# SpectacularAI/HybVIO

Hardware: AMD Instinct MI355X
Metric: VIO frames/sec at 752x480 stereo, 200 KLT features; pyramid+KLT HBM GB/s (higher is better)
Workload: dtype u8/int16 pixels, int32/int64 sums, f32 solve (tracker); f64 (EKF); 1 GPU; C3: 752x480 stereo, 200 pts -- the whole frame chained on one stream per sequence: 2 pyramid builds, temporal LK from predicted positions, 2-point rotation RANSAC on its output, stereo LK, GFTT key points every 2nd frame (HIP tracker), then the HIP EKF from the device mean: 20 track visits (triangulation + prepareVisualUpdate + chi2 gate; track lengths 5 + Geometric(0.2) <= 21 stereo poses = 20 .~; sequences_per_gpu=4096, engines_per_gpu=4, parallelism=replicas x1 (no collective)

## Files before the change

hybvio_amd/csrc/vu_prepare.hip:

```cpp
#include <stdlib.h>

#include "ekf_device.hpp"

#pragma clang fp contract(fast)

namespace hv {
__device__ long long g_vu_stamp[40];
__device__ long long g_tri_stamp[64];
#ifdef HV_EKF_PHASE_STAMPS
#define VU_STAMP(i) do { if (blockIdx.x == 0 && threadIdx.x == 0) g_vu_stamp[i] = (long long)__builtin_readcyclecounter(); } while (0)
#define TRI_STAMP(i) do { if (blockIdx.x == 0 && threadIdx.x == 0) g_tri_stamp[i] = (long long)__builtin_readcyclecounter(); } while (0)
#else
#define VU_STAMP(i) do { } while (0)
#define TRI_STAMP(i) do { } while (0)
#endif
namespace {

constexpr int VT_LATENCY = 768, VT_THROUGHPUT = 384;
constexpr int MAXP_ALL = 42;
constexpr int MAXP_SMALL = 22;
constexpr int MAXP_REC = 24;
constexpr int MAXNP = 21;
constexpr int POSE_WORDS = 51;
constexpr int ITER_WORDS = 26;
// ... 246 lines not shown
    mv3(dd, col, mapped);
    const int dst = j < 7 ? j : j < 14 ? 7 * ind1 + (j - 7) : dDim;
    if (!(j < 7 && ind1 == 0)) {
#pragma unroll
        for (int r = 0; r < 3; ++r) s_dpfi[r * ncol + dst] = mapped[r];
    }
    if (tid == 0) {
#pragma unroll
        for (int k = 0; k < 3; ++k) { pfi[k] = ip3[k]; pfw[k] = pf[k]; }
#pragma unroll
        for (int r = 0; r < 3; ++r)
#pragma unroll
            for (int c = 0; c < 3; ++c) R0T[3 * r + c] = R0[3 * c + r];
        scal[1] = 0.0; scal[2] = 1e10;
        s_flag[0] = 0;
    }
}

template <int MAXP, bool LONG = false>
struct VuLds {
    static constexpr int MAXC = MAXP * 7 + 1, MOT_STRIDE = 13;
    static constexpr int MAXPAIRS = 14 * MAXP - 7;
    static constexpr int LONG_T = (HV_GATE_TIGHT_ROWS + 2) * HV_GATE_TIGHT_ROWS, LONG_HS = (7 * MAXNP + 1) * HV_GATE_TIGHT_ROWS;
    static_assert(LONG_T == 7224 && LONG_HS == 12432, "the long gate's areas as the kernels were measured with");
    static constexpr int TRAIL = 0, IT = TRAIL + MAXP * POSE_WORDS, DPFI = IT + MAXP * ITER_WORDS, FEAT = DPFI + 3 * MAXC,
                         SMALL = FEAT + MAXP * 4, DPF = SMALL + 64, P0 = DPF + MAXNP * 21, MOT = P0 + 7 * MAXP * 9 + 7 * 9,
                         OWN = MOT + MAXPAIRS * MOT_STRIDE, LIN = OWN + MAXC * 9, LIN_END = LIN + 3 * MAXP * 9 + 32,
                         INTS = (LONG && LONG_T + LONG_HS > LIN_END) ? LONG_T + LONG_HS : LIN_END,
                         TOTAL = INTS + (MAXNP + 3 + 4 + MAXC + 1) / 2 + 1;
    static_assert(!LONG || P0 <= LONG_T, "the sources of the Jacobian's factors must lie below the region they are copied to");
    static constexpr int HS_DOUBLES = INTS - P0, T_DOUBLES = P0;
    static constexpr size_t BYTES = sizeof(double) * TOTAL;
};
static_assert(VuLds<42, true>::BYTES <= LDS_CU_BYTES, "the long build must fit one CU's LDS");

template <int MAXP, bool LONG = false>
struct VuRecLds {
    static constexpr int MAXC = MAXP * 7 + 1, MOT_STRIDE = 13;
    static constexpr int LONG_T = VuLds<MAXP, LONG>::LONG_T, LONG_HS = VuLds<MAXP, LONG>::LONG_HS;
    static constexpr int TRAIL = 0, IT = 0, FEAT = IT + MAXP * ITER_WORDS, DPF = FEAT + MAXP * 4, DPFI = DPF + MAXP * 21, SMALL = DPFI + 4,
                         SMALL_END = SMALL + 64;
    static constexpr int SHORT_T = lds_stride(48 + 1) * 48, SHORT_HS = ((7 * (MAXP_REC / 2) + 1 + 3) & ~3) * 48;
    static_assert(SHORT_T == 2352 && SHORT_HS == 4224, "the short gate's areas as the kernels were measured with");
    static constexpr int P0 = LONG ? LONG_T : SHORT_T;
    static constexpr int MOT = P0, OWN = P0, LIN = P0;
    static constexpr int INTS = LONG ? LONG_T + LONG_HS : P0 + SHORT_HS;
    static constexpr int TOTAL = INTS + (MAXNP + 3 + 4 + MAXC + 1) / 2 + 1;
    static constexpr int HS_DOUBLES = INTS - P0, T_DOUBLES = P0;
    static_assert(SMALL_END <= P0, "the record's copies must fit in front of the staged Jacobian");
    static constexpr size_t BYTES = sizeof(double) * TOTAL;
};
static_assert(VuRecLds<MAXP_REC>::BYTES + 32 <= 42 * 1280, "three record-fed short-class gates per CU");

__device__ __forceinline__ void prepare_pose_part(const double *pose, const double *pfw, double *o)
{
    const double pt[3] = {pfw[0] - pose[0], pfw[1] - pose[1], pfw[2] - pose[2]};
    double pfc[3], ipH[3], dip[9];
    mv3(pose + 3, pt, pfc);
    inverse_depth(pfc, ipH, dip);
    o[16] = pfc[2] == 0 ? 1.0 : pfc[2] < 0 ? 2.0 : 0.0;
    o[14] = ipH[0]; o[15] = ipH[1];
#pragma unroll
    for (int r = 0; r < 2; ++r)
#pragma unroll
        for (int c = 0; c < 3; ++c) o[3 * r + c] = dip[3 * r] * pose[3 + c] + dip[3 * r + 1] * pose[6 + c] + dip[3 * r + 2] * pose[9 + c];
#pragma unroll
    for (int jq = 0; jq < 4; ++jq) {
        const double *dR = pose + 12 + 9 * jq;
        double a1[3], b1[3], b2[3];
        mv3(dR, pt, a1);
        mTv3(dR, pose + 48, b1);
        mv3(pose + 3, b1, b2);
#pragma unroll
        for (int r = 0; r < 2; ++r) o[6 + 4 * r + jq] = dip[3 * r] * (a1[0] + b2[0]) + dip[3 * r + 1] * (a1[1] + b2[1]) + dip[3 * r + 2] * (a1[2] + b2[2]);
    }
}

__device__ __forceinline__ bool vu_admission(const VuPrepareArgs &a, const int b, const size_t rec, const int np_rec, const bool no_track)
{
    const int tid = threadIdx.x;
    const bool quota_used = a.success_counter && a.success_counter[b] >= a.max_successful;
    if (a.spec_tracks > 0) {
        if ((int)blockIdx.y < a.cursor[b]) return true;
        if (!quota_used && a.epoch[rec] == a.success_counter[b]) return true;
    }
    if (a.np_hi > 0 && np_rec >= 2 && np_rec <= a.np && (np_rec < a.np_lo || np_rec > a.np_hi)) {
        if (tid == 0) {
            if (a.class_inactive && a.active) a.active[rec] = 0;
            if (a.long_list && np_rec > a.np_hi) a.long_list[atomicAdd(a.long_count, 1)] = (int)rec;
        }
        return true;
    }
    if (a.np_hi > 0 && a.np_lo > 2 && no_track) {
        if (a.class_inactive && a.active && tid == 0) a.active[rec] = 0;
        return true;
    }
    if (quota_used) {
        if (tid == 0) {
            a.status[2 * rec] = HV_TRI_NOT_VISITED; a.status[2 * rec + 1] = HV_TRI_NOT_VISITED;
            if (a.active) a.active[rec] = 0;
            if (a.gate_status) a.gate_status[rec] = 1;
            if (a.spec_tracks > 0) {
                if (a.chi2) a.chi2[rec] = 0.0;
                a.pf[3 * rec] = 0.0; a.pf[3 * rec + 1] = 0.0; a.pf[3 * rec + 2] = 0.0;
            }
        }
        return true;
    }
    if (no_track) {
        if (tid == 0) {
            a.status[2 * rec] = HV_TRI_NOT_VISITED; a.status[2 * rec + 1] = HV_TRI_NOT_VISITED;
            if (a.active) a.active[rec] = 0;
            if (a.gate_status) a.gate_status[rec] = 1;
            if (a.rows_out) a.rows_out[rec] = 0;
            if (a.spec_tracks > 0) a.epoch[rec] = a.success_counter[b];
        }
        return true;
    }
    return false;
}

template <int VT, int MAXP, int FUSED, bool MAP = false, bool REC = false>
__device__ __forceinline__ void vu_prepare_body(const VuPrepareArgs &a, const int bx )
{
    static_assert(!REC || (FUSED == 1 || FUSED == 3), "record-fed builds are gate builds");
    using Lay = std::conditional_t<REC, VuRecLds<MAXP, FUSED == 3>, VuLds<MAXP, FUSED == 3>>;
    constexpr int MOT_STRIDE = Lay::MOT_STRIDE;
    extern __shared__ __attribute__((aligned(16))) double vu_lds[];
// ... 310 lines not shown
        double *M = s_small + 40, *pf0 = s_small + 49;
        if (tid == 0 && !(MAP && map_track)) {
            int status = HV_TRI_OK;
            if (a.linear) {  }
            else if (!s_flag[0]) status = HV_TRI_NO_CONVERGENCE;
            else if (scal[1] < a.rcond_threshold) status = HV_TRI_BAD_COND;
            if (status == HV_TRI_OK && !a.linear) {
                double d[9], q[3], w[3], Ml[9];
                inverse_depth(pfi, q, d);
                mv3(R0T, q, w);
#pragma unroll
                for (int k = 0; k < 3; ++k) { pfw[k] = w[k] + p0[k]; pf0[k] = q[k]; }
                if (pfw[0] == p0[0] && pfw[1] == p0[1] && pfw[2] == p0[2]) status = HV_TRI_UNKNOWN_PROBLEM;
                mm3(R0T, d, Ml);
#pragma unroll
                for (int k = 0; k < 9; ++k) M[k] = Ml[k];
            }
            s_flag[1] = status;
            s_flag[2] = 0;
        }
        __syncthreads();
        status = s_flag[1];
        if (status == HV_TRI_OK) {
            if (tid < ncol && !a.linear) {
                const int j = tid;
                double u[3] = {0, 0, 0}, v[3];
                if (j >= 3 && j < 7) mTv3(s_trail + 12 + 9 * (j - 3), pf0, u);
                const double cur[3] = {s_dpfi[j], s_dpfi[ncol + j], s_dpfi[2 * ncol + j]};
                mv3(M, cur, v);
#pragma unroll
                for (int r = 0; r < 3; ++r) s_dpfi[r * ncol + j] = u[r] + v[r] + (j == r ? 1.0 : 0.0);
            }
            if (tid < nt) {
                const double *cur = s_trail + tid * POSE_WORDS;
                const double d[3] = {pfw[0] - cur[0], pfw[1] - cur[1], pfw[2] - cur[2]};
                if (cur[9] * d[0] + cur[10] * d[1] + cur[11] * d[2] < 0) atomicOr(&s_flag[2], 1);
            }
            __syncthreads();
            if (s_flag[2]) status = HV_TRI_BEHIND;
        }
        if (!(MAP && map_track)) {
            const double dx = pfw[0] - p0[0], dy = pfw[1] - p0[1], dz = pfw[2] - p0[2], depth = sqrt(dx * dx + dy * dy + dz * dz);
            if (depth < a.min_dist || depth > a.max_dist) status = HV_TRI_BAD_DEPTH;
        }
        with_derivatives = status == HV_TRI_OK;
        if (with_derivatives)
            for (int i = tid; i < n * 21; i += VT) {
                const int k = i / 21, e = i - 21 * k, r = e / 7, c = e - 7 * r;
                double v = s_dpfi[r * ncol + 7 * k + c];
                if (a.stereo) v += s_dpfi[r * ncol + 7 * (k + n) + c];
                s_dpf[i] = v;
            }
        VU_STAMP(28);
        if (tid < nt) prepare_pose_part(s_trail + tid * POSE_WORDS, pfw, s_it + tid * ITER_WORDS);
        __syncthreads();
        VU_STAMP(29);
    }
    auto sft_col = [&](int c) -> double { return REC ? s_dpfi[c] : s_dpfi[c * ncol + dDim]; };
    const int rows = 2 * nt;
    if constexpr (FUSED != 0) {
        int prep = 0;
        for (int i = 0; i < nt && prep == 0; ++i) prep = (int)s_it[i * ITER_WORDS + 16];
        const double pf_out[3] = {pfw[0], pfw[1], pfw[2]};
        if (!(status == HV_TRI_OK && prep == 0)) {
            if (tid == 0) {
                st_out[0] = status; st_out[1] = prep;
                if (a.active) a.active[rec] = 0;
                if (a.gate_status) a.gate_status[rec] = 1;
                if (a.chi2) a.chi2[rec] = 0.0;
                if (a.spec_tracks > 0) a.epoch[rec] = a.success_counter[b];
#pragma unroll
                for (int k = 0; k < 3; ++k) a.pf[3 * rec + k] = pf_out[k];
            }
            return;
        }
        if (tid == 0) {
            st_out[0] = HV_TRI_OK; st_out[1] = 0;
            if (a.active) a.active[rec] = 1;
#pragma unroll
            for (int k = 0; k < 3; ++k) a.pf[3 * rec + k] = pf_out[k];
        }
        constexpr bool STRUCT = FUSED == 3;
        constexpr bool STAGED = FUSED == 1;
        const int na = 7 * n + 1, na4 = (na + 3) & ~3, ti = (rows + 15) >> 4;
        int Rs = lds_stride(rows + 1);
        constexpr int T_CAP = FUSED == 3 ? Lay::LONG_T : Lay::T_DOUBLES, REGION = FUSED == 3 ? Lay::LONG_HS : Lay::HS_DOUBLES;
        if (STRUCT && Rs * rows > T_CAP) Rs = lds_stride_tight(rows + 1);
        const int nrp = 16 * ti;
        double *Hs = vu_lds + (FUSED == 3 ? Lay::LONG_T : Lay::P0);
        const int f4s = na, nslots_g = VT / ((na + 63) & ~63);
        double *f_O4 = Hs, *f_DV = f_O4 + 4 * rows, *f_F4 = f_DV + 7 * rows, *f_WF = f_F4 + 4 * f4s, *f_FA = f_WF + 4 * na,
               *f_DWF = f_FA + 4 * rows, *f_FWF = f_DWF + 4 * rows, *f_WFp = f_FWF + 16, *f_G = f_WFp + 3 * na * nslots_g;
        const int g_cap = REGION - (int)(f_G - Hs);
        int *s_acol = s_flag + 4;
        if (tid < na) {
            int col = SFT;
            if (tid < 7 * n) {
                const int q = tid / 7, comp = tid - 7 * q;
                int ip, io;
                pos_ori(s_idx[q], ip, io);
                col = comp < 3 ? ip + comp : io + comp - 3;
            }
            s_acol[tid] = col;
            a.acol[rec * a.na_max + tid] = col;
        }
        if constexpr (STRUCT) {
            if (tid < nt) {
                const double *o = s_it + tid * ITER_WORDS;
                double *o4 = f_O4 + 8 * tid, *dv = f_DV + 14 * tid;
#pragma unroll
                for (int c = 0; c < 3; ++c) { o4[c] = o[c]; o4[4 + c] = o[3 + c]; }
                o4[3] = a.est_shift ? -s_feat[4 * tid + 2] : 0.0; o4[7] = a.est_shift ? -s_feat[4 * tid + 3] : 0.0;
#pragma unroll
                for (int comp = 0; comp < 7; ++comp) {
                    dv[comp] = comp < 3 ? -o[comp] : o[6 + comp - 3];
// ... 121 lines not shown
            if (a.spec_tracks > 0) a.epoch[rec] = a.success_counter[b];
        }
        return;
    }
    double *H = a.H + rec * rows_max * N;
    int *s_colmap = reinterpret_cast<int *>(s_p0);
    for (int c = tid; c < N; c += VT) {
        int code = -1;
        for (int q = 0; q < n; ++q) {
            int ip, io;
            pos_ori(s_idx[q], ip, io);
            if (c >= ip && c < ip + 3) code = 8 * q + (c - ip);
            else if (c >= io && c < io + 4) code = 8 * q + 3 + (c - io);
        }
        s_colmap[c] = code;
    }
    __syncthreads();
    const unsigned inv_nt = (unsigned)((0x100000000ull + (unsigned)nt - 1) / (unsigned)nt);
    for (int w = tid; w < N * nt; w += VT) {
        const int c = (int)__umulhi((unsigned)w, inv_nt), i = w - c * nt;
        const int code = s_colmap[c], k = code >> 3, comp = code & 7;
        const bool sft = c == 19 && with_derivatives && a.est_shift;
        const double *o = s_it + i * ITER_WORDS;
        double h0 = 0.0, h1 = 0.0;
        if (code >= 0) {
            if (k == i % n) {
                if (comp < 3) { h0 = -o[comp]; h1 = -o[3 + comp]; }
                else { h0 = o[6 + comp - 3]; h1 = o[10 + comp - 3]; }
            }
            if (with_derivatives) {
                const double *dp = s_dpf + 21 * k + comp;
                h0 += o[0] * dp[0] + o[1] * dp[7] + o[2] * dp[14];
                h1 += o[3] * dp[0] + o[4] * dp[7] + o[5] * dp[14];
            }
        } else if (sft) {
            const double t0 = s_dpfi[dDim], t1 = s_dpfi[ncol + dDim], t2 = s_dpfi[2 * ncol + dDim];
            h0 = o[0] * t0 + o[1] * t1 + o[2] * t2 - s_feat[4 * i + 2];
            h1 = o[3] * t0 + o[4] * t1 + o[5] * t2 - s_feat[4 * i + 3];
        }
        if (MAP && map_track && c >= map_off && c < map_off + 3) { h0 += o[c - map_off]; h1 += o[3 + c - map_off]; }
        *reinterpret_cast<double2 *>(H + (size_t)c * rows + 2 * i) = double2{h0, h1};
    }
    if (tid < nt) {
        const double *o = s_it + tid * ITER_WORDS;
#pragma unroll
        for (int r = 0; r < 2; ++r) {
            const size_t e = rec * rows_max + 2 * tid + r;
            if (a.f) a.f[e] = o[14 + r];
            a.v[e] = (a.y ? a.y[e] : 0.0) - o[14 + r];
        }
    }
    VU_STAMP(30);
    if (tid == 0) {
        int prep = 0;
        for (int i = 0; i < nt && prep == 0; ++i) prep = (int)s_it[i * ITER_WORDS + 16];
        st_out[0] = status; st_out[1] = prep;
        if (a.active) a.active[rec] = ((status == HV_TRI_OK || (MAP && map_track)) && prep == 0) ? 1 : 0;
        if (a.gate_status) a.gate_status[rec] = 1;
        if (a.spec_tracks > 0) a.epoch[rec] = a.success_counter[b];
#pragma unroll
        for (int k = 0; k < 3; ++k) a.pf[3 * rec + k] = pfw[k];
    }
}

constexpr int TRI_ITW = 28;
struct TriLds {
    int trail, it, dpfi, feat, small, scr, lsum, tot, ints, total;
    __host__ __device__ TriLds(int ntm)
    {
        trail = 0; it = trail + ntm * POSE_WORDS; dpfi = it + ntm * TRI_ITW; feat = dpfi + 3 * (7 * ntm + 1);
        small = feat + 4 * ntm; scr = small + 72; lsum = scr + 7 * ntm * 9; tot = lsum + 32; ints = tot + 64;
        total = ints + (MAXNP + 3 + 4 + 1) / 2 + 1;
    }
};

__device__ __forceinline__ double strided_sum(const double *base, int stride, int n, int part, int parts)
{
    double a0 = 0.0, a1 = 0.0, a2 = 0.0, a3 = 0.0;
    int k = part;
    for (; k + 3 * parts < n; k += 4 * parts) {
        a0 += base[(size_t)k * stride]; a1 += base[(size_t)(k + parts) * stride];
        a2 += base[(size_t)(k + 2 * parts) * stride]; a3 += base[(size_t)(k + 3 * parts) * stride];
    }
    for (; k < n; k += parts) a0 += base[(size_t)k * stride];
    return (a0 + a1) + (a2 + a3);
}

template <int NT>
__device__ __forceinline__ void vu_tri_body(const VuPrepareArgs &a, const int b)
{
    extern __shared__ __attribute__((aligned(16))) double vu_lds[];
    const int tid = threadIdx.x;
    const size_t rec = (size_t)b;
    const int np_rec = __builtin_amdgcn_readfirstlane(a.np_rec ? a.np_rec[rec] : a.np);
    if (np_rec < 2 || np_rec > a.np) return;
    if (a.np_hi > 0 && (np_rec < a.np_lo || np_rec > a.np_hi)) return;
    if (a.success_counter && a.success_counter[b] >= a.max_successful) return;
    const int n = np_rec, ncam = a.stereo ? 2 : 1, nt = n * ncam, N = a.n;
    const int nt_max = a.np * ncam;
    const int dDim = nt * 7, ncol = dDim + 1;
    const int np_carve = a.np_hi > 0 && a.np_hi < a.np ? a.np_hi : a.np;
    const TriLds L(np_carve * ncam);
    double *s_trail = vu_lds + L.trail, *s_it = vu_lds + L.it, *s_dpfi = vu_lds + L.dpfi, *s_feat = vu_lds + L.feat;
    double *s_small = vu_lds + L.small, *s_scr = vu_lds + L.scr, *s_L = vu_lds + L.lsum, *s_tot = vu_lds + L.tot;
    int *s_idx = reinterpret_cast<int *>(vu_lds + L.ints), *s_flag = s_idx + MAXNP + 3;
    const double *m = a.m + (size_t)b * N;
    double *pfi = s_small, *pfw = s_small + 3, *R0T = s_small + 18, *scal = s_small + 36, *sums13 = s_small + 52;
    auto sync = [] { lds_barrier(); };
    TRI_STAMP(0);
    if (tid < n) s_idx[tid] = a.pose_index[rec * a.np + tid];
    if (tid < nt) {
#pragma unroll
        for (int k = 0; k < 2; ++k) {
            s_feat[4 * tid + k] = a.features[(rec * nt_max + tid) * 2 + k];
            s_feat[4 * tid + 2 + k] = a.velocities[(rec * nt_max + tid) * 2 + k];
        }
    }
    sync();
    TRI_STAMP(1);
    if (tid < nt) trail_pose_record(a, m, s_idx, tid, n, s_trail + tid * POSE_WORDS);
    for (int i = tid; i < 3 * ncol; i += NT) s_dpfi[i] = 0.0;
    sync();
    TRI_STAMP(2);
    const double *p0 = s_trail;
    const int ind1 = a.stereo ? nt / 2 - 1 : nt - 1;
    if (tid < 15) two_camera_start(a, tid, ind1, ncol, dDim, s_trail, s_feat, s_dpfi, pfi, pfw, R0T, scal, s_flag);
    sync();
    TRI_STAMP(3);
    const double *Lm = s_L;
    auto update_col = [&](int j, const double *own, bool is_sft, const double (&X)[9], const double (&step)[3]) {
        const double d0 = s_dpfi[j], d1 = s_dpfi[ncol + j], d2 = s_dpfi[2 * ncol + j];
        double v[9];
#pragma unroll
        for (int e = 0; e < 9; ++e) v[e] = (Lm[e] * d0 + Lm[9 + e] * d1) + Lm[18 + e] * d2;
        double dEe[3] = {v[0], v[1], v[2]}, dM[9] = {v[3], v[4], v[5], v[4], v[6], v[7], v[5], v[7], v[8]};
        if (!is_sft) {
#pragma unroll
            for (int k = 0; k < 3; ++k) dEe[k] += own[k];
            dM[0] += own[3]; dM[1] += own[4]; dM[2] += own[5]; dM[4] += own[6]; dM[5] += own[7]; dM[8] += own[8];
            dM[3] = dM[1]; dM[6] = dM[2]; dM[7] = dM[5];
        } else {
#pragma unroll
            for (int k = 0; k < 3; ++k) dEe[k] += Lm[27 + k];
        }
        double t1[3], t2[3], t3[3];
        mv3(dM, step, t1);
        mv3(X, t1, t2);
        mv3(X, dEe, t3);
#pragma unroll
        for (int r = 0; r < 3; ++r) s_dpfi[r * ncol + j] += t2[r] - t3[r];
    };
    constexpr int PARTS_L = NT >= 240 ? 8 : NT >= 120 ? 4 : 2;
    constexpr int PARTS_T = NT >= 252 ? 4 : NT >= 126 ? 2 : 1;
    const int NC = 4 * nt, NPp = 3 * (nt - 1), NQ = 4 * (nt - 1);
    for (int it = 0; it < a.gn_iters; ++it) {
#define TRI_IT_STAMP(k) do { if (it < 5) TRI_STAMP(4 + 10 * it + (k)); } while (0)
        TRI_IT_STAMP(0);
        if (tid < nt) {
            const double *cur = s_trail + tid * POSE_WORDS;
            double *o = s_it + tid * TRI_ITW;
            double C[9], t[3], d[3], h[3];
            mm3(cur + 3, R0T, C);
#pragma unroll
            for (int k = 0; k < 3; ++k) d[k] = p0[k] - cur[k];
            mv3(cur + 3, d, t);
            const double pfiab[3] = {pfi[0], pfi[1], 1.0};
            mv3(C, pfiab, h);
#pragma unroll
            for (int k = 0; k < 3; ++k) h[k] += pfi[2] * t[k];
            const double ih2 = 1.0 / h[2], ih2sq = ih2 * ih2;
#pragma unroll
            for (int k = 0; k < 9; ++k) o[k] = C[k];
#pragma unroll
            for (int k = 0; k < 3; ++k) { o[9 + k] = t[k]; o[12 + k] = h[k]; o[23 + k] = d[k]; }
            o[26] = ih2;
#pragma unroll
            for (int r = 0; r < 2; ++r) {
#pragma unroll
                for (int c = 0; c < 2; ++c) o[15 + 3 * r + c] = -ih2 * C[3 * r + c] + h[r] * ih2sq * C[6 + c];
                o[15 + 3 * r + 2] = -t[r] * ih2 + h[r] * ih2sq * t[2];
                o[21 + r] = s_feat[4 * tid + r] - h[r] * ih2;
            }
        }
        sync();
        TRI_IT_STAMP(1);
        if (tid < 52) {
            const int k = tid >> 2, part = tid & 3;
            const int r = k / 3, c = k - 3 * r;
            const int x0 = k < 9 ? 15 + r : k < 12 ? 15 + (k - 9) : 21, y0 = k < 9 ? 15 + c : 21;
            const int dx = k < 12 ? 3 : 1, dy = k < 9 ? 3 : 1;
            double acc = 0.0, acc2 = 0.0;
            int i = part;
            for (; i + 4 < nt; i += 8) {
                const double *o = s_it + i * TRI_ITW, *o2 = o + 4 * TRI_ITW;
                acc += o[x0] * o[y0] + o[x0 + dx] * o[y0 + dy];
                acc2 += o2[x0] * o2[y0] + o2[x0 + dx] * o2[y0 + dy];
            }
            if (i < nt) { const double *o = s_it + i * TRI_ITW; acc += o[x0] * o[y0] + o[x0 + dx] * o[y0 + dy]; }
            acc += acc2;
            acc += __shfl_xor(acc, 1);
            acc += __shfl_xor(acc, 2);
            if (part == 0) sums13[k] = acc;
        }
        {
            const int t0 = NT > 64 ? tid - 64 : tid, tstep = NT > 64 ? NT - 64 : NT;
            if (t0 >= 0)
                for (int task = t0; task < 3 * nt; task += tstep) {
                    const int i = task / 3, u = task - 3 * i;
                    const double *o = s_it + i * TRI_ITW;
                    const double dh[3] = {u < 2 ? o[u] : o[9], u < 2 ? o[3 + u] : o[10], u < 2 ? o[6 + u] : o[11]};
                    double e3[3] = {0, 0, 0}, m9[9] = {0, 0, 0, 0, 0, 0, 0, 0, 0};
                    pair_sums<0>(o, dh, nullptr, nullptr, 0.0, 0.0, e3, m9, o + 26);
                    double *dst = s_scr + task * 9;
                    dst[0] = e3[0]; dst[1] = e3[1]; dst[2] = e3[2];
                    dst[3] = m9[0]; dst[4] = m9[1]; dst[5] = m9[2]; dst[6] = m9[4]; dst[7] = m9[5]; dst[8] = m9[8];
                }
        }
        sync();
        TRI_IT_STAMP(2);
        if (tid < 30 * PARTS_L) {
            const int sigma = tid / PARTS_L, part = tid - sigma * PARTS_L;
            double acc;
            if (sigma < 27) {
                const int u = sigma / 9, e = sigma - 9 * u;
                acc = strided_sum(s_scr + u * 9 + e, 27, nt, part, PARTS_L);
            } else {
                const int r = sigma - 27;
                acc = 0.0;
                for (int q = part; q < nt; q += PARTS_L)
                    acc += s_it[q * TRI_ITW + 15 + r] * s_feat[4 * q + 2] + s_it[q * TRI_ITW + 18 + r] * s_feat[4 * q + 3];
            }
#pragma unroll
            for (int o = 1; o < PARTS_L; o <<= 1) acc += __shfl_xor(acc, o);
            if (part == 0) s_L[sigma] = acc;
        }
        double X[9], step[3];
        {
            double ETE[9], Ee[3];
#pragma unroll
            for (int q = 0; q < 9; ++q) ETE[q] = sums13[q];
#pragma unroll
            for (int q = 0; q < 3; ++q) Ee[q] = sums13[9 + q];
            inv3sym(ETE, X);
            mv3(X, Ee, step);
        }
        sync();
        TRI_IT_STAMP(3);
        const int gC = (NC + 63) >> 6, gP = (NPp + 63) >> 6, gQ = (NQ + 63) >> 6;
        for (int grp = tid >> 6; grp < gC + gP + gQ; grp += NT / 64) {
            const int lane_ = tid & 63;
            const int ty = grp < gC ? 0 : grp < gC + gP ? 1 : 2;
            const int e_in = (grp - (ty == 0 ? 0 : ty == 1 ? gC : gC + gP)) * 64 + lane_;
            if (e_in >= (ty == 0 ? NC : ty == 1 ? NPp : NQ)) continue;
            const int e = e_in + (ty == 0 ? 0 : ty == 1 ? NC : NC + NPp);
            if (ty == 0) {
                const int q = e / nt, i = e - q * nt;
                const double *cur = s_trail + i * POSE_WORDS, *dR0 = s_trail + 12 + 9 * q, *o = s_it + i * TRI_ITW;
                double dC[9], dt[3], dp0[3], dh[3], e3[3] = {0, 0, 0}, m9[9] = {0, 0, 0, 0, 0, 0, 0, 0, 0};
                mmT3(cur + 3, dR0, dC);
                mTv3(dR0, s_trail + 48, dp0);
                const double dd[3] = {-dp0[0], -dp0[1], -dp0[2]};
                mv3(cur + 3, dd, dt);
                if (i == 0) {
                    double a1[9];
                    mm3(dR0, R0T, a1);
#pragma unroll
                    for (int k = 0; k < 9; ++k) dC[k] += a1[k];
                    dt[0] = 0.0; dt[1] = 0.0; dt[2] = 0.0;
                }
#pragma unroll
                for (int r = 0; r < 3; ++r) dh[r] = (dC[3 * r] * pfi[0] + dC[3 * r + 1] * pfi[1] + dC[3 * r + 2]) + pfi[2] * dt[r];
                pair_sums<1>(o, dh, dC, dt, 0.0, 0.0, e3, m9, o + 26);
                double *dst = s_scr + ((3 + q) * nt + i) * 9;
                dst[0] = e3[0]; dst[1] = e3[1]; dst[2] = e3[2];
                dst[3] = m9[0]; dst[4] = m9[1]; dst[5] = m9[2]; dst[6] = m9[4]; dst[7] = m9[5]; dst[8] = m9[8];
            } else if (ty == 1) {
                const int e2 = e - NC, c = e2 / (nt - 1), i = 1 + e2 - c * (nt - 1);
                const double *cur = s_trail + i * POSE_WORDS, *o = s_it + i * TRI_ITW;
                const double dt[3] = {cur[3 + c], cur[6 + c], cur[9 + c]};
                const double dh[3] = {pfi[2] * dt[0], pfi[2] * dt[1], pfi[2] * dt[2]};
                double e3[3] = {0, 0, 0}, m9[9] = {0, 0, 0, 0, 0, 0, 0, 0, 0};
                pair_sums<2>(o, dh, nullptr, dt, 0.0, 0.0, e3, m9, o + 26);
                const double r9[9] = {e3[0], e3[1], e3[2], m9[0], m9[1], m9[2], m9[4], m9[5], m9[8]};
                double *dst = s_scr + (c * nt + i) * 9;
                double own[9];
#pragma unroll
                for (int k = 0; k < 9; ++k) { dst[k] = r9[k]; own[k] = -r9[k]; }
                update_col(7 * i + c, own, false, X, step);
            } else {
                const int e2 = e - NC - NPp, q = e2 / (nt - 1), i = 1 + e2 - q * (nt - 1);
                const double *cur = s_trail + i * POSE_WORDS, *dR = cur + 12 + 9 * q, *o = s_it + i * TRI_ITW;
                double dC[9], dt[3], dpi[3], t1[3], t2[3], dh[3], e3[3] = {0, 0, 0}, m9[9] = {0, 0, 0, 0, 0, 0, 0, 0, 0};
                mm3(dR, R0T, dC);
                mTv3(dR, cur + 48, dpi);
                mv3(dR, o + 23, t1);
                mv3(cur + 3, dpi, t2);
#pragma unroll
                for (int k = 0; k < 3; ++k) dt[k] = t1[k] + t2[k];
#pragma unroll
                for (int r = 0; r < 3; ++r) dh[r] = (dC[3 * r] * pfi[0] + dC[3 * r + 1] * pfi[1] + dC[3 * r + 2]) + pfi[2] * dt[r];
                pair_sums<1>(o, dh, dC, dt, 0.0, 0.0, e3, m9, o + 26);
                const double own[9] = {e3[0], e3[1], e3[2], m9[0], m9[1], m9[2], m9[4], m9[5], m9[8]};
                update_col(7 * i + 3 + q, own, false, X, step);
            }
        }
        sync();
        TRI_IT_STAMP(4);
        if (tid < 63 * PARTS_T) {
            const int sigma = tid / PARTS_T, part = tid - sigma * PARTS_T;
            const int comp = sigma / 9, en = sigma - 9 * comp, first = comp < 3 ? 1 : 0;
            double acc = strided_sum(s_scr + ((size_t)comp * nt + first) * 9 + en, 9, nt - first, part, PARTS_T);
#pragma unroll
            for (int o = 1; o < PARTS_T; o <<= 1) acc += __shfl_xor(acc, o);
            if (part == 0) s_tot[sigma] = acc;
        }
        sync();
        TRI_IT_STAMP(5);
        if (tid < 8) {
            const bool sft = tid == 7;
            if (!sft || a.est_shift) update_col(sft ? dDim : tid, s_tot + 9 * (sft ? 0 : tid), sft, X, step);
        } else if (tid == NT - 1) {
#pragma unroll
            for (int k = 0; k < 3; ++k) pfi[k] -= step[k];
            const double J = 0.5 * sums13[12] / (a.conv_r * a.conv_r), Jd = fabs((J - scal[2]) / J);
            scal[2] = J;
            if (Jd < a.conv_threshold) s_flag[0] = 1;
        }
        sync();
        TRI_IT_STAMP(6);
#undef TRI_IT_STAMP
        if (s_flag[0]) break;
    }
    TRI_STAMP(54);
    double *M = s_small + 40, *pf0 = s_small + 49;
    if (tid == 0) {
        int status = HV_TRI_OK;
        if (a.gn_iters > 0) {
            double ETE[9], Xl[9];
#pragma unroll
            for (int q = 0; q < 9; ++q) ETE[q] = sums13[q];
            inv3sym(ETE, Xl);
            scal[1] = 1.0 / (norm1_3(ETE) * norm1_3(Xl));
        }
        if (!s_flag[0]) status = HV_TRI_NO_CONVERGENCE;
        else if (scal[1] < a.rcond_threshold) status = HV_TRI_BAD_COND;
        if (status == HV_TRI_OK) {
            double d[9], q[3], w[3], Ml[9];
            inverse_depth(pfi, q, d);
            mv3(R0T, q, w);
#pragma unroll
            for (int k = 0; k < 3; ++k) { pfw[k] = w[k] + p0[k]; pf0[k] = q[k]; }
            if (pfw[0] == p0[0] && pfw[1] == p0[1] && pfw[2] == p0[2]) status = HV_TRI_UNKNOWN_PROBLEM;
            mm3(R0T, d, Ml);
#pragma unroll
            for (int k = 0; k < 9; ++k) M[k] = Ml[k];
        }
        s_flag[1] = status;
        s_flag[2] = 0;
    }
    sync();
    TRI_STAMP(55);
    int status = s_flag[1];
    double *recp = a.tri_rec + rec * (size_t)a.tri_stride;
    const VuTriRec R(a.np, nt_max);
    {
        const int t0 = NT > 64 ? tid - (NT - 64) : tid;
        if (t0 >= 0 && t0 < nt) {
            const double *pose = s_trail + t0 * POSE_WORDS;
            double *o = recp + VuTriRec::POSE * t0;
            const double pt[3] = {pfw[0] - pose[0], pfw[1] - pose[1], pfw[2] - pose[2]};
            if (status == HV_TRI_OK && pose[9] * pt[0] + pose[10] * pt[1] + pose[11] * pt[2] < 0) atomicOr(&s_flag[2], 1);
            double pfc[3], ipH[3], dip[9];
            mv3(pose + 3, pt, pfc);
            inverse_depth(pfc, ipH, dip);
            const double cls = pfc[2] == 0 ? 1.0 : pfc[2] < 0 ? 2.0 : 0.0;
            o[16] = cls;
            s_it[t0 * TRI_ITW + 16] = cls;
            o[14] = ipH[0]; o[15] = ipH[1];
#pragma unroll
            for (int r = 0; r < 2; ++r)
#pragma unroll
                for (int c = 0; c < 3; ++c) o[3 * r + c] = dip[3 * r] * pose[3 + c] + dip[3 * r + 1] * pose[6 + c] + dip[3 * r + 2] * pose[9 + c];
#pragma unroll
            for (int jq = 0; jq < 4; ++jq) {
                const double *dR = pose + 12 + 9 * jq;
                double a1[3], b1[3], b2[3];
                mv3(dR, pt, a1);
                mTv3(dR, pose + 48, b1);
                mv3(pose + 3, b1, b2);
#pragma unroll
                for (int r = 0; r < 2; ++r) o[6 + 4 * r + jq] = dip[3 * r] * (a1[0] + b2[0]) + dip[3 * r + 1] * (a1[1] + b2[1]) + dip[3 * r + 2] * (a1[2] + b2[2]);
            }
        }
    }
    if (status == HV_TRI_OK) {
        auto world = [&](int j, int r) -> double {
            double u = 0.0;
            if (j >= 3 && j < 7) { const double *dR = s_trail + 12 + 9 * (j - 3); u = dR[r] * pf0[0] + dR[3 + r] * pf0[1] + dR[6 + r] * pf0[2]; }
            const double v = M[3 * r] * s_dpfi[j] + M[3 * r + 1] * s_dpfi[ncol + j] + M[3 * r + 2] * s_dpfi[2 * ncol + j];
            return u + v + (j == r ? 1.0 : 0.0);
        };
        const int nlan = NT > 64 ? NT - 64 : NT;
        if (tid < nlan)
            for (int i = tid; i < n * 21; i += nlan) {
                const int k = i / 21, e = i - 21 * k, r = e / 7, c = e - 7 * r;
                double v = world(7 * k + c, r);
                if (a.stereo) v += world(7 * (k + n) + c, r);
                recp[R.dpf + i] = v;
            }
        if (tid < 3) recp[R.sft + tid] = a.est_shift ? world(dDim, tid) : 0.0;
    }
    sync();
    TRI_STAMP(56);
    if (tid == 0) {
        if (status == HV_TRI_OK && s_flag[2]) status = HV_TRI_BEHIND;
        {
            const double dx = pfw[0] - p0[0], dy = pfw[1] - p0[1], dz = pfw[2] - p0[2], depth = sqrt(dx * dx + dy * dy + dz * dz);
            if (depth < a.min_dist || depth > a.max_dist) status = HV_TRI_BAD_DEPTH;
        }
        int prep = 0;
        for (int i = 0; i < nt && prep == 0; ++i) prep = (int)s_it[i * TRI_ITW + 16];
        recp[R.prep] = (double)prep;
        a.status[2 * rec] = status;
#pragma unroll
        for (int k = 0; k < 3; ++k) a.pf[3 * rec + k] = pfw[k];
    }
    TRI_STAMP(57);
}

__global__ __launch_bounds__(64) void vu_tri_kernel(VuPrepareArgs a)
{
    int b = blockIdx.x;
    if (a.rec_list) { if (b >= *a.rec_count) return; b = a.rec_list[b]; }
    else if (a.order) b = __builtin_amdgcn_readfirstlane(a.order[blockIdx.x]);
    vu_tri_body<64>(a, b);
}
__global__ __launch_bounds__(256) void vu_tri_kernel_x4(VuPrepareArgs a)
{
    int b = blockIdx.x;
    if (a.rec_list) { if (b >= *a.rec_count) return; b = a.rec_list[b]; }
    else if (a.order) b = __builtin_amdgcn_readfirstlane(a.order[blockIdx.x]);
    vu_tri_body<256>(a, b);
}
__global__ __launch_bounds__(128) void vu_tri_kernel_x2(VuPrepareArgs a)
{
    int b = blockIdx.x;
    if (a.rec_list) { if (b >= *a.rec_count) return; b = a.rec_list[b]; }
    else if (a.order) b = __builtin_amdgcn_readfirstlane(a.order[blockIdx.x]);
    vu_tri_body<128>(a, b);
}

__global__ __launch_bounds__(VT_LATENCY, 3) void vu_prepare_kernel(VuPrepareArgs a) { vu_prepare_body<VT_LATENCY, MAXP_ALL, 0>(a, blockIdx.x); }
__global__ __launch_bounds__(VT_THROUGHPUT, 4) void vu_prepare_kernel_2percu(VuPrepareArgs a)
{
    vu_prepare_body<VT_THROUGHPUT, MAXP_SMALL, 0>(a, blockIdx.x);
}
__global__ __launch_bounds__(VT_LATENCY, 3) void vu_prepare_map_kernel(VuPrepareArgs a) { vu_prepare_body<VT_LATENCY, MAXP_ALL, 0, true>(a, blockIdx.x); }
__global__ __launch_bounds__(VT_LATENCY, 3) void vu_gate_kernel(VuPrepareArgs a) { vu_prepare_body<VT_LATENCY, MAXP_ALL, 1>(a, blockIdx.x); }
__global__ __launch_bounds__(VT_THROUGHPUT, 4) void vu_gate_kernel_2percu(VuPrepareArgs a)
{
    const int b = a.order ? __builtin_amdgcn_readfirstlane(a.order[blockIdx.x]) : (int)blockIdx.x;
    vu_prepare_body<VT_THROUGHPUT, MAXP_SMALL, 1>(a, b);
}

constexpr int VT_REC = 256;
__global__ __launch_bounds__(VT_REC, 3) void vu_gate_rec_kernel(VuPrepareArgs a)
{
    const int b = a.order ? __builtin_amdgcn_readfirstlane(a.order[blockIdx.x]) : (int)blockIdx.x;
    vu_prepare_body<VT_REC, MAXP_REC, 1, false, true>(a, b);
}
__global__ __launch_bounds__(VT_LATENCY, 3) void vu_gate_long_rec_kernel(VuPrepareArgs a)
{
    int b = blockIdx.x;
    if (a.rec_list) { if (b >= *a.rec_count) return; b = a.rec_list[b]; }
    vu_prepare_body<VT_LATENCY, MAXP_ALL, 3, false, true>(a, b);
// ... 192 lines not shown
```

Measured before the change: 153,900 frames/s.

## Hold loop-invariant pair Jacobians in registers; ballot first failing pose; odd LDS stride

The triangulation Gauss-Newton pair phase is moved into a helper. On the 128- and 256-thread kernels, it forms the per-pose rotation and translation derivatives (dC, dt) once on iteration zero and keeps them in registers for later iterations, so they are not recomputed every iteration. The first failing pose's projection class is now found with a wavefront ballot and written to a shared flag, replacing serial scans over the LDS by thread 0. The per-pose LDS stride drops from 28 to 27, an odd value meant to avoid bank conflicts for consecutive lanes. In exchange, register pressure rises by up to 36 doubles per thread, and the ballot assumes all of a track's poses fit in one wavefront.

```diff
diff --git a/hybvio_amd/csrc/vu_prepare.hip b/hybvio_amd/csrc/vu_prepare.hip
--- a/hybvio_amd/csrc/vu_prepare.hip
+++ b/hybvio_amd/csrc/vu_prepare.hip
@@ -322,13 +322,14 @@
 };
 static_assert(VuRecLds<MAXP_REC>::BYTES + 32 <= 42 * 1280, "three record-fed short-class gates per CU");
 
-__device__ __forceinline__ void prepare_pose_part(const double *pose, const double *pfw, double *o)
+__device__ __forceinline__ double prepare_pose_part(const double *pose, const double *pfw, double *o)
 {
     const double pt[3] = {pfw[0] - pose[0], pfw[1] - pose[1], pfw[2] - pose[2]};
     double pfc[3], ipH[3], dip[9];
     mv3(pose + 3, pt, pfc);
     inverse_depth(pfc, ipH, dip);
-    o[16] = pfc[2] == 0 ? 1.0 : pfc[2] < 0 ? 2.0 : 0.0;
+    const double cls = pfc[2] == 0 ? 1.0 : pfc[2] < 0 ? 2.0 : 0.0;
+    o[16] = cls;
     o[14] = ipH[0]; o[15] = ipH[1];
 #pragma unroll
     for (int r = 0; r < 2; ++r)
@@ -344,6 +345,7 @@
 #pragma unroll
         for (int r = 0; r < 2; ++r) o[6 + 4 * r + jq] = dip[3 * r] * (a1[0] + b2[0]) + dip[3 * r + 1] * (a1[1] + b2[1]) + dip[3 * r + 2] * (a1[2] + b2[2]);
     }
+    return cls;
 }
 
 __device__ __forceinline__ bool vu_admission(const VuPrepareArgs &a, const int b, const size_t rec, const int np_rec, const bool no_track)
@@ -760,7 +762,11 @@
                 s_dpf[i] = v;
             }
         VU_STAMP(28);
-        if (tid < nt) prepare_pose_part(s_trail + tid * POSE_WORDS, pfw, s_it + tid * ITER_WORDS);
+        if (tid < nt) {
+            const double cls = prepare_pose_part(s_trail + tid * POSE_WORDS, pfw, s_it + tid * ITER_WORDS);
+            const unsigned long long failing = __ballot(cls != 0.0);
+            if (failing ? tid == __ffsll(failing) - 1 : tid == 0) s_flag[3] = (int)cls;
+        }
         __syncthreads();
         VU_STAMP(29);
     }
@@ -768,7 +774,8 @@
     const int rows = 2 * nt;
     if constexpr (FUSED != 0) {
         int prep = 0;
-        for (int i = 0; i < nt && prep == 0; ++i) prep = (int)s_it[i * ITER_WORDS + 16];
+        if constexpr (REC) { for (int i = 0; i < nt && prep == 0; ++i) prep = (int)s_it[i * ITER_WORDS + 16]; }
+        else prep = s_flag[3];
         const double pf_out[3] = {pfw[0], pfw[1], pfw[2]};
         if (!(status == HV_TRI_OK && prep == 0)) {
             if (tid == 0) {
@@ -996,8 +1003,7 @@
     }
     VU_STAMP(30);
     if (tid == 0) {
-        int prep = 0;
-        for (int i = 0; i < nt && prep == 0; ++i) prep = (int)s_it[i * ITER_WORDS + 16];
+        const int prep = s_flag[3];
         st_out[0] = status; st_out[1] = prep;
         if (a.active) a.active[rec] = ((status == HV_TRI_OK || (MAP && map_track)) && prep == 0) ? 1 : 0;
         if (a.gate_status) a.gate_status[rec] = 1;
@@ -1007,7 +1013,8 @@
     }
 }
 
-constexpr int TRI_ITW = 28;
+constexpr int TRI_ITW = 27;
+static_assert(TRI_ITW % 2 == 1 && TRI_ITW > ITER_WORDS && POSE_WORDS % 2 == 1, "odd per-pose strides: conflict-free for consecutive lanes");
 struct TriLds {
     int trail, it, dpfi, feat, small, scr, lsum, tot, ints, total;
     __host__ __device__ TriLds(int ntm)
@@ -1028,6 +1035,108 @@
     }
     for (; k < n; k += parts) a0 += base[(size_t)k * stride];
     return (a0 + a1) + (a2 + a3);
+}
+
+struct TriPairCtx { int tid, it, nt; const double *s_trail, *s_it; double *s_scr; const double *pfi, *R0T; };
+template <bool HELD, class UpdateCol>
+__device__ __forceinline__ void tri_pair_task(const TriPairCtx &pc, const int grp, double (&held_dC)[9], double (&held_dt)[3],
+                                              const double (&X)[9], const double (&step)[3], const UpdateCol &update_col)
+{
+    const int tid = pc.tid, it = pc.it, nt = pc.nt;
+    const double *s_trail = pc.s_trail, *s_it = pc.s_it, *pfi = pc.pfi, *R0T = pc.R0T;
+    double *s_scr = pc.s_scr;
+    const int NC = 4 * nt, NPp = 3 * (nt - 1), NQ = 4 * (nt - 1);
+    const int gC = (NC + 63) >> 6, gP = (NPp + 63) >> 6;
+    const int lane_ = tid & 63;
+    const int ty = grp < gC ? 0 : grp < gC + gP ? 1 : 2;
+    const int e_in = (grp - (ty == 0 ? 0 : ty == 1 ? gC : gC + gP)) * 64 + lane_;
+    if (e_in >= (ty == 0 ? NC : ty == 1 ? NPp : NQ)) return;
+    const int e = e_in + (ty == 0 ? 0 : ty == 1 ? NC : NC + NPp);
+    const bool form = !HELD || it == 0;
+    if (ty == 0) {
+        const int q = e / nt, i = e - q * nt;
+        const double *cur = s_trail + i * POSE_WORDS, *dR0 = s_trail + 12 + 9 * q, *o = s_it + i * TRI_ITW;
+        double dC[9], dt[3], dh[3], e3[3] = {0, 0, 0}, m9[9] = {0, 0, 0, 0, 0, 0, 0, 0, 0};
+        if (form) {
+            double dp0[3];
+            mmT3(cur + 3, dR0, dC);
+            mTv3(dR0, s_trail + 48, dp0);
+            const double dd[3] = {-dp0[0], -dp0[1], -dp0[2]};
+            mv3(cur + 3, dd, dt);
+            if (i == 0) {
+                double a1[9];
+                mm3(dR0, R0T, a1);
+#pragma unroll
+                for (int k = 0; k < 9; ++k) dC[k] += a1[k];
+                dt[0] = 0.0; dt[1] = 0.0; dt[2] = 0.0;
+            }
+            if constexpr (HELD) {
+#pragma unroll
+                for (int k = 0; k < 9; ++k) held_dC[k] = dC[k];
+#pragma unroll
+                for (int k = 0; k < 3; ++k) held_dt[k] = dt[k];
+            }
+        } else if constexpr (HELD) {
+#pragma unroll
+            for (int k = 0; k < 9; ++k) dC[k] = held_dC[k];
+#pragma unroll
+            for (int k = 0; k < 3; ++k) dt[k] = held_dt[k];
+        }
+#pragma unroll
+        for (int r = 0; r < 3; ++r) dh[r] = (dC[3 * r] * pfi[0] + dC[3 * r + 1] * pfi[1] + dC[3 * r + 2]) + pfi[2] * dt[r];
+        pair_sums<1>(o, dh, dC, dt, 0.0, 0.0, e3, m9, o + 26);
+        double *dst = s_scr + ((3 + q) * nt + i) * 9;
+        dst[0] = e3[0]; dst[1] = e3[1]; dst[2] = e3[2];
+        dst[3] = m9[0]; dst[4] = m9[1]; dst[5] = m9[2]; dst[6] = m9[4]; dst[7] = m9[5]; dst[8] = m9[8];
+    } else if (ty == 1) {
+        const int e2 = e - NC, c = e2 / (nt - 1), i = 1 + e2 - c * (nt - 1);
+        const double *cur = s_trail + i * POSE_WORDS, *o = s_it + i * TRI_ITW;
+        const double dt[3] = {cur[3 + c], cur[6 + c], cur[9 + c]};
+        const double dh[3] = {pfi[2] * dt[0], pfi[2] * dt[1], pfi[2] * dt[2]};
+        double e3[3] = {0, 0, 0}, m9[9] = {0, 0, 0, 0, 0, 0, 0, 0, 0};
+        pair_sums<2>(o, dh, nullptr, dt, 0.0, 0.0, e3, m9, o + 26);
+        const double r9[9] = {e3[0], e3[1], e3[2], m9[0], m9[1], m9[2], m9[4], m9[5], m9[8]};
+        double *dst = s_scr + (c * nt + i) * 9;
+        double own[9];
+#pragma unroll
+        for (int k = 0; k < 9; ++k) { dst[k] = r9[k]; own[k] = -r9[k]; }
+        update_col(7 * i + c, own, false, X, step);
+    } else {
+        const int e2 = e - NC - NPp, q = e2 / (nt - 1), i = 1 + e2 - q * (nt - 1);
+        const double *cur = s_trail + i * POSE_WORDS, *dR = cur + 12 + 9 * q, *o = s_it + i * TRI_ITW;
+        double dC[9], dt[3], dh[3], e3[3] = {0, 0, 0}, m9[9] = {0, 0, 0, 0, 0, 0, 0, 0, 0};
+        if (form) {
+            double dpi[3], t1[3], t2[3];
+            mm3(dR, R0T, dC);
+            mTv3(dR, cur + 48, dpi);
+            mv3(dR, o + 23, t1);
+            mv3(cur + 3, dpi, t2);
+#pragma unroll
+            for (int k = 0; k < 3; ++k) dt[k] = t1[k] + t2[k];
+            if constexpr (HELD) {
+#pragma unroll
+                for (int k = 0; k < 9; ++k) held_dC[k] = dC[k];
+#pragma unroll
+                for (int k = 0; k < 3; ++k) held_dt[k] = dt[k];
+            }
+        } else if constexpr (HELD) {
+#pragma unroll
+            for (int k = 0; k < 9; ++k) dC[k] = held_dC[k];
+#pragma unroll
+            for (int k = 0; k < 3; ++k) dt[k] = held_dt[k];
+        }
+#pragma unroll
+        for (int r = 0; r < 3; ++r) dh[r] = (dC[3 * r] * pfi[0] + dC[3 * r + 1] * pfi[1] + dC[3 * r + 2]) + pfi[2] * dt[r];
+        pair_sums<1>(o, dh, dC, dt, 0.0, 0.0, e3, m9, o + 26);
+        const double own[9] = {e3[0], e3[1], e3[2], m9[0], m9[1], m9[2], m9[4], m9[5], m9[8]};
+        update_col(7 * i + 3 + q, own, false, X, step);
+    }
+}
+
+constexpr int tri_pair_rounds(int nt, int threads)
+{
+    const int groups = (4 * nt + 63) / 64 + (3 * (nt - 1) + 63) / 64 + (4 * (nt - 1) + 63) / 64, waves = threads / 64;
+    return (groups + waves - 1) / waves;
 }
 
 template <int NT>
@@ -1042,6 +1151,7 @@
     if (a.success_counter && a.success_counter[b] >= a.max_successful) return;
     const int n = np_rec, ncam = a.stereo ? 2 : 1, nt = n * ncam, N = a.n;
     const int nt_max = a.np * ncam;
+    static_assert(MAXP_ALL <= 64, "the poses of a track are lanes of ONE wavefront (the ballot for the first failing pose)");
     const int dDim = nt * 7, ncol = dDim + 1;
     const int np_carve = a.np_hi > 0 && a.np_hi < a.np ? a.np_hi : a.np;
     const TriLds L(np_carve * ncam);
@@ -1097,6 +1207,10 @@
     constexpr int PARTS_L = NT >= 240 ? 8 : NT >= 120 ? 4 : 2;
     constexpr int PARTS_T = NT >= 252 ? 4 : NT >= 126 ? 2 : 1;
     const int NC = 4 * nt, NPp = 3 * (nt - 1), NQ = 4 * (nt - 1);
+    constexpr int HOLD_ROUNDS = NT == 128 ? tri_pair_rounds(MAXP_REC, 128) : NT == 256 ? tri_pair_rounds(MAXP_ALL, 256) : 0;
+    static_assert(NT != 128 || HOLD_ROUNDS == 3, "vu_tri_kernel_x2: the short class's pair phase is three rounds");
+    static_assert(NT != 256 || HOLD_ROUNDS == 2, "vu_tri_kernel_x4: the long class's pair phase is two rounds");
+    double hold_dC[HOLD_ROUNDS > 0 ? HOLD_ROUNDS : 1][9], hold_dt[HOLD_ROUNDS > 0 ? HOLD_ROUNDS : 1][3];
     for (int it = 0; it < a.gn_iters; ++it) {
 #define TRI_IT_STAMP(k) do { if (it < 5) TRI_STAMP(4 + 10 * it + (k)); } while (0)
         TRI_IT_STAMP(0);
@@ -1191,63 +1305,13 @@
         sync();
         TRI_IT_STAMP(3);
         const int gC = (NC + 63) >> 6, gP = (NPp + 63) >> 6, gQ = (NQ + 63) >> 6;
-        for (int grp = tid >> 6; grp < gC + gP + gQ; grp += NT / 64) {
-            const int lane_ = tid & 63;
-            const int ty = grp < gC ? 0 : grp < gC + gP ? 1 : 2;
-            const int e_in = (grp - (ty == 0 ? 0 : ty == 1 ? gC : gC + gP)) * 64 + lane_;
-            if (e_in >= (ty == 0 ? NC : ty == 1 ? NPp : NQ)) continue;
-            const int e = e_in + (ty == 0 ? 0 : ty == 1 ? NC : NC + NPp);
-            if (ty == 0) {
-                const int q = e / nt, i = e - q * nt;
-                const double *cur = s_trail + i * POSE_WORDS, *dR0 = s_trail + 12 + 9 * q, *o = s_it + i * TRI_ITW;
-                double dC[9], dt[3], dp0[3], dh[3], e3[3] = {0, 0, 0}, m9[9] = {0, 0, 0, 0, 0, 0, 0, 0, 0};
-                mmT3(cur + 3, dR0, dC);
-                mTv3(dR0, s_trail + 48, dp0);
-                const double dd[3] = {-dp0[0], -dp0[1], -dp0[2]};
-                mv3(cur + 3, dd, dt);
-                if (i == 0) {
-                    double a1[9];
-                    mm3(dR0, R0T, a1);
-#pragma unroll
-                    for (int k = 0; k < 9; ++k) dC[k] += a1[k];
-                    dt[0] = 0.0; dt[1] = 0.0; dt[2] = 0.0;
-                }
-#pragma unroll
-                for (int r = 0; r < 3; ++r) dh[r] = (dC[3 * r] * pfi[0] + dC[3 * r + 1] * pfi[1] + dC[3 * r + 2]) + pfi[2] * dt[r];
-                pair_sums<1>(o, dh, dC, dt, 0.0, 0.0, e3, m9, o + 26);
-                double *dst = s_scr + ((3 + q) * nt + i) * 9;
-                dst[0] = e3[0]; dst[1] = e3[1]; dst[2] = e3[2];
-                dst[3] = m9[0]; dst[4] = m9[1]; dst[5] = m9[2]; dst[6] = m9[4]; dst[7] = m9[5]; dst[8] = m9[8];
-            } else if (ty == 1) {
-                const int e2 = e - NC, c = e2 / (nt - 1), i = 1 + e2 - c * (nt - 1);
-                const double *cur = s_trail + i * POSE_WORDS, *o = s_it + i * TRI_ITW;
-                const double dt[3] = {cur[3 + c], cur[6 + c], cur[9 + c]};
-                const double dh[3] = {pfi[2] * dt[0], pfi[2] * dt[1], pfi[2] * dt[2]};
-                double e3[3] = {0, 0, 0}, m9[9] = {0, 0, 0, 0, 0, 0, 0, 0, 0};
-                pair_sums<2>(o, dh, nullptr, dt, 0.0, 0.0, e3, m9, o + 26);
-                const double r9[9] = {e3[0], e3[1], e3[2], m9[0], m9[1], m9[2], m9[4], m9[5], m9[8]};
-                double *dst = s_scr + (c * nt + i) * 9;
-                double own[9];
-#pragma unroll
-                for (int k = 0; k < 9; ++k) { dst[k] = r9[k]; own[k] = -r9[k]; }
-                update_col(7 * i + c, own, false, X, step);
-            } else {
-                const int e2 = e - NC - NPp, q = e2 / (nt - 1), i = 1 + e2 - q * (nt - 1);
-                const double *cur = s_trail + i * POSE_WORDS, *dR = cur + 12 + 9 * q, *o = s_it + i * TRI_ITW;
-                double dC[9], dt[3], dpi[3], t1[3], t2[3], dh[3], e3[3] = {0, 0, 0}, m9[9] = {0, 0, 0, 0, 0, 0, 0, 0, 0};
-                mm3(dR, R0T, dC);
-                mTv3(dR, cur + 48, dpi);
-                mv3(dR, o + 23, t1);
-                mv3(cur + 3, dpi, t2);
-#pragma unroll
-                for (int k = 0; k < 3; ++k) dt[k] = t1[k] + t2[k];
-#pragma unroll
-                for (int r = 0; r < 3; ++r) dh[r] = (dC[3 * r] * pfi[0] + dC[3 * r + 1] * pfi[1] + dC[3 * r + 2]) + pfi[2] * dt[r];
-                pair_sums<1>(o, dh, dC, dt, 0.0, 0.0, e3, m9, o + 26);
-                const double own[9] = {e3[0], e3[1], e3[2], m9[0], m9[1], m9[2], m9[4], m9[5], m9[8]};
-                update_col(7 * i + 3 + q, own, false, X, step);
-            }
-        }
+        const TriPairCtx pc{tid, it, nt, s_trail, s_it, s_scr, pfi, R0T};
+        static_assert(HOLD_ROUNDS <= 3, "one call per held round below");
+        const int grp0 = tid >> 6, groups = gC + gP + gQ;
+        if constexpr (HOLD_ROUNDS > 0) { if (grp0 < groups) tri_pair_task<true>(pc, grp0, hold_dC[0], hold_dt[0], X, step, update_col); }
+        if constexpr (HOLD_ROUNDS > 1) { if (grp0 + NT / 64 < groups) tri_pair_task<true>(pc, grp0 + NT / 64, hold_dC[1], hold_dt[1], X, step, update_col); }
+        if constexpr (HOLD_ROUNDS > 2) { if (grp0 + 2 * (NT / 64) < groups) tri_pair_task<true>(pc, grp0 + 2 * (NT / 64), hold_dC[2], hold_dt[2], X, step, update_col); }
+        for (int grp = grp0 + HOLD_ROUNDS * (NT / 64); grp < groups; grp += NT / 64) tri_pair_task<false>(pc, grp, hold_dC[0], hold_dt[0], X, step, update_col);
         sync();
         TRI_IT_STAMP(4);
         if (tid < 63 * PARTS_T) {
@@ -1319,7 +1383,10 @@
             inverse_depth(pfc, ipH, dip);
             const double cls = pfc[2] == 0 ? 1.0 : pfc[2] < 0 ? 2.0 : 0.0;
             o[16] = cls;
-            s_it[t0 * TRI_ITW + 16] = cls;
+            {
+                const unsigned long long failing = __ballot(cls != 0.0);
+                if (failing ? t0 == __ffsll(failing) - 1 : t0 == 0) s_flag[3] = (int)cls;
+            }
             o[14] = ipH[0]; o[15] = ipH[1];
 #pragma unroll
             for (int r = 0; r < 2; ++r)
@@ -1362,9 +1429,7 @@
             const double dx = pfw[0] - p0[0], dy = pfw[1] - p0[1], dz = pfw[2] - p0[2], depth = sqrt(dx * dx + dy * dy + dz * dz);
             if (depth < a.min_dist || depth > a.max_dist) status = HV_TRI_BAD_DEPTH;
         }
-        int prep = 0;
-        for (int i = 0; i < nt && prep == 0; ++i) prep = (int)s_it[i * TRI_ITW + 16];
-        recp[R.prep] = (double)prep;
+        recp[R.prep] = (double)s_flag[3];
         a.status[2 * rec] = status;
 #pragma unroll
         for (int k = 0; k < 3; ++k) a.pf[3 * rec + k] = pfw[k];
```

Result: no change. 154,700 frames/s, median of 6 (+0.5%).
